# QData/LaMP

Measured on AMD Instinct MI355X. Metric: forward samples/sec, reuters d512 2+2L 4h, higher is better.
Workload: dtype f32

## Files before the change

### lamp_amd/csrc/chain.hip

```cpp
#include "lamp_asm.h"

namespace lamp {

namespace {
constexpr int ROWS = 16;
constexpr int BK = 32;

}

struct ChainGemm {
    const float* W[3];
    const float* Wp[3];
    const float* Wq[3];
    const float* bias[3];
    float* C[3];
    int nseg, N, K;
    int64_t ldw, ldc;
    int relu;
    int src;
    int dst;
    int add_dst;
};
struct ChainLN {
    const float* g;
// ... 453 lines not shown
    const int tid = threadIdx.x, lane = tid & 63;
    const int wave = __builtin_amdgcn_readfirstlane(tid >> 6);
    const int l15 = lane & 15, hi = lane >> 4;
    const int64_t row0 = int64_t(blockIdx.x) * ROWS;
    const int rows_m = int(p.M - row0 < ROWS ? p.M - row0 : ROWS);
    const unsigned lds0 = unsigned(reinterpret_cast<uintptr_t>((lds_ptr)smem));
    const int d = p.d, dff = p.has_ffn ? p.w1.N : 0;
    const int x_floats = ROWS * d, h_floats = ROWS * p.hw;
    const int c_floats = x_floats + h_floats;
    const int c_g1 = c_floats, c_be1 = c_g1 + d, c_g2 = c_be1 + d, c_be2 = c_g2 + d, c_b2 = c_be2 + d, c_b1 = c_b2 + d;
    const int c_res = c_b1 + dff, c_wout = c_res + (p.ln1.res ? ROWS * d : 0);
    auto buf_b = [&](int which) { return lds0 + (which ? unsigned(x_floats) * 4u : 0u); };
    auto buf_f = [&](int which) { return smem + (which ? x_floats : 0); };
    auto buf_w = [&](int which) { return which ? p.hw : d; };

    int pc = 0;
    auto first = [&]() { return (wave - pc) & (WAVES - 1); };
    auto load_rows = [&](const float* src, int64_t ld, int width, int which) {
        const __amdgpu_buffer_rsrc_t rs = rsrc_u(src + row0 * ld, (uint64_t(rows_m - 1) * uint64_t(ld) + uint64_t(width)) * 4u);
        const int ppr = width / 256, n = ROWS * ppr;
        float* dst = buf_f(which);
        const int rl = buf_w(which);
        for (int k = first(); k < n; k += WAVES) {
            const int r = k / ppr, part = k - r * ppr;
            const unsigned voff = unsigned(r) * unsigned(ld) * 4u + unsigned(part * 64 + (lane ^ r)) * 16u;
            lds_dma16(rs, dst + r * rl + part * 256, r < rows_m ? voff : OOB, 0);
        }
        pc += n;
    };
    auto load_vec = [&](const float* src, int n_floats, int at) {
        const __amdgpu_buffer_rsrc_t rs = rsrc_u(src, uint64_t(n_floats) * 4u);
        const int n = n_floats / 256;
        for (int k = first(); k < n; k += WAVES) lds_dma16(rs, smem + at + k * 256, unsigned(k * 64 + lane) * 16u, 0);
        pc += n;
    };
    auto load_mod_rows = [&](const float* table, int mod, int at) {
        const __amdgpu_buffer_rsrc_t rs = rsrc_u(table, uint64_t(mod) * uint64_t(d) * 4u);
        const int ppr = d / 256, n = ROWS * ppr;
        for (int k = first(); k < n; k += WAVES) {
            const int r = k / ppr, part = k - r * ppr;
            const unsigned src_row = unsigned(row0 + r) % unsigned(mod);
            lds_dma16(rs, smem + at + r * d + part * 256, r < rows_m ? (src_row * unsigned(d) + unsigned(part * 64 + lane) * 4u) * 4u : OOB, 0);
        }
        pc += n;
    };
    if (p.in_x) load_rows(p.in_x, d, d, 0);
    load_rows(p.in_h, p.ld_h, p.k_h, 1);
    load_vec(p.ln1.g, d, c_g1);
    load_vec(p.ln1.b, d, c_be1);
    if (p.ln1.res) load_mod_rows(p.ln1.res, p.ln1.r_mod, c_res);
    const ChainLN& lnl = p.has_ffn ? p.ln2 : p.ln1;
    if (p.has_ffn) {
        load_vec(p.ln2.g, d, c_g2);
        load_vec(p.ln2.b, d, c_be2);
        load_vec(p.w2.bias[0], d, c_b2);
        load_vec(p.w1.bias[0], dff, c_b1);
    }
    if (lnl.w_out) load_mod_rows(lnl.w_out, lnl.n_labels, c_wout);
    wait_vmcnt<0>();
    wg_barrier();

    unsigned a_off[2][2];
#pragma unroll
    for (int o = 0; o < 2; ++o)
#pragma unroll
        for (int c = 0; c < 2; ++c) a_off[o][c] = unsigned(((o * 8 + c * 4 + hi) ^ l15) << 4);

#ifdef LAMP_TUNING
    unsigned long long gt[3][4] = {};
    int gt_i = 0;
#endif
    auto gemm = [&](const ChainGemm& g, int bias_at) {
        CHAIN_STAMP(0);
        const int nk = g.K / BK, npass = g.N / PASS_COLS, total = npass * nk;
        const unsigned w_bytes = unsigned(g.N) * unsigned(g.K) * 4u;
        u32x4 rsW = raw_rsrc(g.Wp[0], w_bytes);
        unsigned f_voff[2][NB];
#pragma unroll
        for (int c = 0; c < 2; ++c)
#pragma unroll
            for (int j = 0; j < NB; ++j) f_voff[c][j] = unsigned((j * nk * 2 + c) * 256 + lane * 4) * 4u;
        const unsigned pass_jump = unsigned(PASS_COLS / 16 - 1) * unsigned(nk) * 2048u + 2048u;
        unsigned s_off = unsigned(wave * (WCOLS / 16)) * unsigned(nk) * 2048u;
        int pt = 0, p_kt = 0, p_wrap = 0;
        auto adv_a = [&]() { ++pt; ++p_kt; p_wrap = p_kt == nk ? 1 : 0; };
        auto adv_b = [&]() { s_off += p_wrap ? pass_jump : 2048u; p_kt = p_wrap ? 0 : p_kt; };
        auto adv_c = [&]() {
#if defined(CHAIN_ABL) && (CHAIN_ABL & 1)
            rsW[2] = 0u;
#else
            rsW[2] = pt < total ? w_bytes : 0u;
#endif
        };
        f32x4 F[DEPTH][2][NB], fa[2][2];
        unsigned a_cur[2][2];
        const unsigned src_b = buf_b(g.src) + unsigned(l15) * unsigned(buf_w(g.src)) * 4u;
#pragma unroll
        for (int o = 0; o < 2; ++o)
#pragma unroll
            for (int c = 0; c < 2; ++c) a_cur[o][c] = src_b + a_off[o][c];
        static_for<0, DEPTH - 1>([&](auto J) {
            constexpr int j = decltype(J)::value;
            sgpr_guard(rsW, s_off);
#pragma unroll
            for (int c = 0; c < 2; ++c)
#pragma unroll
                for (int jb = 0; jb < NB; ++jb) F[j][c][jb] = buffer_read16_untracked(rsW, f_voff[c][jb], s_off);
            adv_a(); adv_b(); adv_c();
        });
#pragma unroll
        for (int c = 0; c < 2; ++c) fa[0][c] = lds_read16(a_cur[0][c]);
        wait_vmcnt<(DEPTH - 2) * NL>();
        wait_lgkmcnt<0>();
        CHAIN_STAMP(1);
        for (int pass = 0; pass < npass; ++pass) {
            const int col0 = pass * PASS_COLS + wave * WCOLS;
            f32x4 acc[NB];
#pragma unroll
            for (int j = 0; j < NB; ++j) acc[j] = f32x4{0.f, 0.f, 0.f, 0.f};
            for (int kt0 = 0; kt0 < nk; kt0 += DEPTH) {
                const unsigned q_next = unsigned(kt0 + DEPTH == nk ? 0 : (kt0 + DEPTH) >> 1) * 256u;
                static_for<0, DEPTH>([&](auto J) {
                    constexpr int j = decltype(J)::value, set = j & 1, setn = (j + 1) & 1;
                    constexpr int jl = (j + DEPTH - 1) % DEPTH;
                    constexpr int a_imm = (j + 1 == DEPTH) ? 0 : ((j + 1) >> 1) * 256;
                    static_for<0, NMF>([&](auto I) {
                        constexpr int i = decltype(I)::value, c = i / (4 * NB), comp = (i % (4 * NB)) / NB, jb = i % NB;
#if !(defined(CHAIN_ABL) && (CHAIN_ABL & 2))
                        acc[jb] = __builtin_amdgcn_mfma_f32_16x16x4f32(F[j][c][jb][comp], fa[set][c][comp], acc[jb], 0, 0, 0);
#else
                        asm volatile("" ::"v"(F[j][c][jb]), "v"(fa[set][c]));
#endif
                        __builtin_amdgcn_sched_barrier(0);
                        if constexpr (i % 2 == 0 && i / 2 < NL) {
                            constexpr int li = i / 2;
#if !(defined(CHAIN_ABL) && (CHAIN_ABL & 16))
                            F[jl][li / NB][li % NB] = buffer_read16_untracked(rsW, f_voff[li / NB][li % NB], s_off);
#endif
                        } else if constexpr (i == 1 || i == 3) {
#if !(defined(CHAIN_ABL) && (CHAIN_ABL & 8))
                            fa[setn][i / 2] = lds_read16_off<a_imm>(a_cur[setn][i / 2]);
#endif
                        } else if constexpr (i == 2 * NL + 1) {
                            adv_a();
                        } else if constexpr (i == 2 * NL + 2) {
                            if constexpr (j == DEPTH - 2) {
                                a_cur[0][0] = src_b + a_off[0][0] + q_next;
                                a_cur[0][1] = src_b + a_off[0][1] + q_next;
                            } else if constexpr (j == DEPTH - 1) {
                                a_cur[1][0] = src_b + a_off[1][0] + q_next;
                                a_cur[1][1] = src_b + a_off[1][1] + q_next;
                            }
                        } else if constexpr (i == 2 * NL + 3) {
                            adv_b();
                        } else if constexpr (i == 2 * NL + 5) {
                            adv_c();
                        } else if constexpr (i == NMF - 1) {
                            asm volatile("s_waitcnt vmcnt(%0) lgkmcnt(0)" ::"n"((DEPTH - 2) * NL) : "memory");
                        }
                        __builtin_amdgcn_sched_barrier(0);
                    });
                });
            }
            if (pass + 1 == npass) wait_vmcnt<0>();
            static_for<0, DEPTH - 1>([&](auto J) {
#pragma unroll
                for (int c = 0; c < 2; ++c)
#pragma unroll
                    for (int jb = 0; jb < NB; ++jb) keep_alive(F[decltype(J)::value][c][jb]);
            });
#pragma unroll
            for (int c = 0; c < 2; ++c) keep_alive(fa[0][c]);
            CHAIN_STAMP(2);
            f32x4 bv[NB], rv[NB];
            unsigned at[NB];
#pragma unroll
            for (int j = 0; j < NB; ++j) {
                const int col = col0 + j * 16 + 4 * hi;
                at[j] = buf_b(g.dst) + unsigned(l15) * unsigned(buf_w(g.dst)) * 4u + unsigned(((col >> 2) ^ l15) << 4);
                bv[j] = lds_read16(bias_at >= 0 ? lds0 + unsigned(bias_at + col) * 4u : at[j]);
                rv[j] = lds_read16(at[j]);
            }
            wait_lgkmcnt<0>();
#pragma unroll
            for (int j = 0; j < NB; ++j) {
                settle(bv[j]);
                settle(rv[j]);
            }
#pragma unroll
            for (int j = 0; j < NB; ++j) {
                const f32x4 b = bias_at >= 0 ? bv[j] : f32x4{0.f, 0.f, 0.f, 0.f};
                float4 v = make_float4(acc[j][0] + b[0], acc[j][1] + b[1], acc[j][2] + b[2], acc[j][3] + b[3]);
                if (g.relu) v = make_float4(fmaxf(v.x, 0.f), fmaxf(v.y, 0.f), fmaxf(v.z, 0.f), fmaxf(v.w, 0.f));
                if (g.add_dst) v = make_float4(v.x + rv[j][0], v.y + rv[j][1], v.z + rv[j][2], v.w + rv[j][3]);
                lds_write16(at[j], f32x4{v.x, v.y, v.z, v.w});
            }
        }
        wait_vmcnt<0>();
        wg_barrier();
        CHAIN_STAMP(3);
#ifdef LAMP_TUNING
        ++gt_i;
#endif
    };

    auto layernorm = [&](const ChainLN& n, int g_at, int be_at) {
        const int nv = d / 4;
        int cq[NV];
#pragma unroll
        for (int i = 0; i < NV; ++i) cq[i] = lane + i * 64 < nv ? lane + i * 64 : nv - 1;
#pragma unroll
        for (int q = 0; q < RPW; ++q) {
            const int r = wave + q * WAVES;
            const bool live = r < rows_m;
            const int64_t row = row0 + (live ? r : 0);
            const unsigned row_b = lds0 + unsigned(r) * unsigned(d) * 4u;
            f32x4 raw[NV], gg[NV], bb[NV], rr[NV], ww[NV];
#pragma unroll
            for (int i = 0; i < NV; ++i) {
                const unsigned self = row_b + unsigned((cq[i] ^ r) << 4);
                raw[i] = lds_read16(self);
                gg[i] = lds_read16(lds0 + unsigned(g_at) * 4u + unsigned(cq[i]) * 16u);
                bb[i] = lds_read16(lds0 + unsigned(be_at) * 4u + unsigned(cq[i]) * 16u);
                rr[i] = lds_read16(n.res ? lds0 + unsigned(c_res + r * d) * 4u + unsigned(cq[i]) * 16u : self);
                ww[i] = lds_read16(n.w_out ? lds0 + unsigned(c_wout + r * d) * 4u + unsigned(cq[i]) * 16u : self);
            }
            wait_lgkmcnt<0>();
#pragma unroll
            for (int i = 0; i < NV; ++i) {
                settle(raw[i]); settle(gg[i]); settle(bb[i]); settle(rr[i]); settle(ww[i]);
            }
            float4 v[NV];
#pragma unroll
            for (int i = 0; i < NV; ++i) {
                const bool in = lane + i * 64 < nv;
                v[i] = in ? make_float4(raw[i].x, raw[i].y, raw[i].z, raw[i].w) : make_float4(0.f, 0.f, 0.f, 0.f);
                if (n.res && in) {
                    v[i].x += rr[i].x; v[i].y += rr[i].y; v[i].z += rr[i].z; v[i].w += rr[i].w;
                }
            }
            float mean, rstd;
            ln_row_stats<NV>(v, lane, nv, d, n.eps, mean, rstd);
            float4* yr = (n.y && live) ? reinterpret_cast<float4*>(n.y + row * d) : nullptr;
            float dot = 0.f;
#pragma unroll
            for (int i = 0; i < NV; ++i) {
                if (lane + i * 64 < nv) {
                    const float4 o = ln_row_apply(v[i], mean, rstd, make_float4(gg[i].x, gg[i].y, gg[i].z, gg[i].w),
                                                  make_float4(bb[i].x, bb[i].y, bb[i].z, bb[i].w));
                    lds_write16(row_b + unsigned((cq[i] ^ r) << 4), f32x4{o.x, o.y, o.z, o.w});
                    if (yr) yr[cq[i]] = o;
                    if (n.w_out) dot += dot4_nocontract(o, make_float4(ww[i].x, ww[i].y, ww[i].z, ww[i].w));
                }
            }
            if (n.w_out) {
                dot = wave64_sum(dot);
                if (lane == 0 && live) n.logits[row] = dot;
            }
        }
        wg_barrier();
    };

#ifdef LAMP_TUNING
    unsigned long long t[6] = {};
    const unsigned long long c_begin = __builtin_readcyclecounter();
    if (p.trace) t[0] = wall_clock64();
#endif
    gemm(p.fc, -1);
#ifdef LAMP_TUNING
    if (p.trace) t[1] = wall_clock64();
#endif
    layernorm(p.ln1, c_g1, c_be1);
#ifdef LAMP_TUNING
    if (p.trace) t[2] = wall_clock64();
#endif
    if (p.has_ffn) {
        gemm(p.w1, c_b1);
#ifdef LAMP_TUNING
        if (p.trace) t[3] = wall_clock64();
#endif
        gemm(p.w2, c_b2);
#ifdef LAMP_TUNING
        if (p.trace) t[4] = wall_clock64();
#endif
        layernorm(p.ln2, c_g2, c_be2);
    }
#ifdef LAMP_TUNING
    if (p.trace && tid == 0) {
        unsigned long long* o = p.trace + size_t(blockIdx.x) * 24;
        t[5] = wall_clock64();
        for (int i = 0; i < 6; ++i) o[i] = t[i];
        o[6] = __builtin_readcyclecounter() - c_begin;
        o[7] = __builtin_amdgcn_s_getreg((31 << 11) | 20);
        for (int gi = 0; gi < 3; ++gi)
            for (int k = 0; k < 4; ++k) o[8 + gi * 4 + k] = gt[gi][k] - c_begin;
    }
#endif
}


template <int NV, int G>
__global__ __launch_bounds__(512, 2) void chain_rows4_kernel(ChainParams p) {
    constexpr int WAVES = 8, R = 4 * G, DEPTH = 4, NMF = 16 * G, RPW = (R + WAVES - 1) / WAVES;
    extern __shared__ __attribute__((aligned(16))) float smem[];
    const int tid = threadIdx.x, lane = tid & 63;
    const int wave = __builtin_amdgcn_readfirstlane(tid >> 6);
    const int l3 = lane & 3;
    const int64_t row0 = int64_t(blockIdx.x) * R;
    const int rows_m = int(p.M - row0 < R ? p.M - row0 : R);
    const unsigned lds0 = unsigned(reinterpret_cast<uintptr_t>((lds_ptr)smem));
    const int d = p.d, dff = p.has_ffn ? p.w1.N : 0;
    const int x_floats = R * d, h_floats = R * p.hw;
    const int c_floats = x_floats + h_floats;
    const int c_g1 = c_floats, c_be1 = c_g1 + d, c_g2 = c_be1 + d, c_be2 = c_g2 + d, c_b2 = c_be2 + d, c_b1 = c_b2 + d;
    const int c_res = p.res_alias ? x_floats + p.k_h : c_b1 + dff, res_ld = p.res_alias ? p.hw : d;
    const int c_wout = p.wout_late ? x_floats : (p.res_alias ? c_b1 + dff : c_res + (p.ln1.res ? R * d : 0));
    auto buf_b = [&](int which) { return lds0 + (which ? unsigned(x_floats) * 4u : 0u); };
    auto buf_f = [&](int which) { return smem + (which ? x_floats : 0); };
    auto buf_w = [&](int which) { return which ? p.hw : d; };

    int pc = 0;
    auto first = [&]() { return (wave - pc) & (WAVES - 1); };
    auto load_rows = [&](const float* src, int64_t ld, int width, int which) {
        const __amdgpu_buffer_rsrc_t rs = rsrc_u(src + row0 * ld, (uint64_t(rows_m - 1) * uint64_t(ld) + uint64_t(width)) * 4u);
        const int ppr = width / 256, n = R * ppr;
        float* dst = buf_f(which);
        const int rl = buf_w(which);
        for (int k = first(); k < n; k += WAVES) {
            const int r = k / ppr, part = k - r * ppr;
            const unsigned voff = unsigned(r) * unsigned(ld) * 4u + unsigned(part * 64 + (lane ^ (r & 15))) * 16u;
            lds_dma16(rs, dst + r * rl + part * 256, r < rows_m ? voff : OOB, 0);
        }
        pc += n;
    };
    auto load_vec = [&](const float* src, int n_floats, int at) {
        const __amdgpu_buffer_rsrc_t rs = rsrc_u(src, uint64_t(n_floats) * 4u);
        const int n = n_floats / 256;
        for (int k = first(); k < n; k += WAVES) lds_dma16(rs, smem + at + k * 256, unsigned(k * 64 + lane) * 16u, 0);
        pc += n;
    };
    auto load_mod_rows = [&](const float* table, int mod, int at, int ld) {
        const __amdgpu_buffer_rsrc_t rs = rsrc_u(table, uint64_t(mod) * uint64_t(d) * 4u);
        const int ppr = d / 256, n = R * ppr;
        for (int k = first(); k < n; k += WAVES) {
            const int r = k / ppr, part = k - r * ppr;
            const unsigned src_row = unsigned(row0 + r) % unsigned(mod);
            lds_dma16(rs, smem + at + r * ld + part * 256, r < rows_m ? (src_row * unsigned(d) + unsigned(part * 64 + lane) * 4u) * 4u : OOB, 0);
        }
        pc += n;
    };
    if (p.in_x) load_rows(p.in_x, d, d, 0);
    load_rows(p.in_h, p.ld_h, p.k_h, 1);
    load_vec(p.ln1.g, d, c_g1);
    load_vec(p.ln1.b, d, c_be1);
    if (p.ln1.res) load_mod_rows(p.ln1.res, p.ln1.r_mod, c_res, res_ld);
    const ChainLN& lnl = p.has_ffn ? p.ln2 : p.ln1;
    if (p.has_ffn) {
        load_vec(p.ln2.g, d, c_g2);
        load_vec(p.ln2.b, d, c_be2);
        load_vec(p.w2.bias[0], d, c_b2);
        load_vec(p.w1.bias[0], dff, c_b1);
    }
    if (lnl.w_out && !p.wout_late) load_mod_rows(lnl.w_out, lnl.n_labels, c_wout, d);
    wait_vmcnt<0>();
    wg_barrier();

#ifdef LAMP_TUNING
    unsigned long long gt[3][4] = {};
    int gt_i = 0;
#endif
    auto gemm = [&](const ChainGemm& g, int bias_at) {
        CHAIN_STAMP(0);
        const int nc = g.K / 16, npass = g.N / 512, total = npass * nc;
        const unsigned w_bytes = unsigned(g.N) * unsigned(g.K) * 4u;
        u32x4 rsW = raw_rsrc(g.Wq[0], w_bytes);
        const unsigned f_voff = unsigned(lane) * 16u;
        const unsigned pass_jump = 7u * unsigned(nc) * 4096u + 4096u;
        unsigned s_off = unsigned(wave) * unsigned(nc) * 4096u;
        int pt = 0, p_kt = 0, p_wrap = 0;
        auto adv_a = [&]() { ++pt; ++p_kt; p_wrap = p_kt == nc ? 1 : 0; };
        auto adv_b = [&]() { s_off += p_wrap ? pass_jump : 4096u; p_kt = p_wrap ? 0 : p_kt; };
        auto adv_c = [&]() {
#if defined(CHAIN_ABL) && (CHAIN_ABL & 1)
            rsW[2] = 0u;
#else
            rsW[2] = pt < total ? w_bytes : 0u;
#endif
        };
        auto wload = [&](f32x4& dst, auto Q) { dst = buffer_read16_untracked_off<decltype(Q)::value * 1024>(rsW, f_voff, s_off); };
        f32x4 F[DEPTH][4];
        float fa[2][G];
        unsigned a_cur[G];
        const unsigned src_b = buf_b(g.src), row_bytes = unsigned(buf_w(g.src)) * 4u;
        const int bq = lane >> 4, be = (lane >> 2) & 3;
        auto a_lane = [&](int gg) { return src_b + unsigned(4 * gg + l3) * row_bytes + unsigned((bq ^ l3) << 4) + unsigned(be) * 4u; };
#pragma unroll
        for (int gg = 0; gg < G; ++gg) a_cur[gg] = a_lane(gg);
        auto aread = [&](auto SET, auto GG, auto J) {
            constexpr int set = decltype(SET)::value, gg = decltype(GG)::value, j = decltype(J)::value;
            fa[set][gg] = lds_read4_off<64 * (j ^ (gg & 3))>(a_cur[gg]);
        };
        static_for<0, DEPTH - 1>([&](auto J) {
            constexpr int j = decltype(J)::value;
            sgpr_guard(rsW, s_off);
            static_for<0, 4>([&](auto Q) { wload(F[j][decltype(Q)::value], Q); });
            adv_a(); adv_b(); adv_c();
        });
        static_for<0, G>([&](auto GG) { aread(std::integral_constant<int, 0>{}, GG, std::integral_constant<int, 0>{}); });
        wait_vmcnt<(DEPTH - 2) * 4>();
        wait_lgkmcnt<0>();
        CHAIN_STAMP(1);
        for (int pass = 0; pass < npass; ++pass) {
            const int col = pass * 512 + wave * 64 + lane;
            f32x4 acc[G];
#pragma unroll
            for (int gg = 0; gg < G; ++gg) acc[gg] = f32x4{0.f, 0.f, 0.f, 0.f};
            for (int kt0 = 0; kt0 < nc; kt0 += DEPTH) {
                const unsigned q_next = unsigned(kt0 + DEPTH == nc ? 0 : (kt0 + DEPTH) >> 2) * 256u;
                static_for<0, DEPTH>([&](auto J) {
                    constexpr int j = decltype(J)::value, set = j & 1, setn = (j + 1) & 1;
                    constexpr int jl = (j + DEPTH - 1) % DEPTH, jn = (j + 1) % DEPTH;
                    static_for<0, NMF>([&](auto I) {
                        constexpr int i = decltype(I)::value, jj = i / (4 * G), q = (i / G) % 4, gg = i % G;
#if !(defined(CHAIN_ABL) && (CHAIN_ABL & 2))
                        acc[gg] = __builtin_amdgcn_mfma_f32_4x4x1f32(fa[set][gg], F[j][q][jj], acc[gg], 4, 4 * q + jj, 0);
#endif
                        __builtin_amdgcn_sched_barrier(0);
                        if constexpr (i < 8 && i % 2 == 0) {
#if !(defined(CHAIN_ABL) && (CHAIN_ABL & 16))
                            wload(F[jl][i / 2], std::integral_constant<int, i / 2>{});
#endif
                        } else if constexpr (i < 2 * G && i % 2 == 1 && i != NMF - 1) {
#if !(defined(CHAIN_ABL) && (CHAIN_ABL & 8))
                            aread(std::integral_constant<int, setn>{}, std::integral_constant<int, i / 2>{}, std::integral_constant<int, jn>{});
#endif
                        } else if constexpr (i == 8) {
                            adv_a();
                        } else if constexpr (i == 10) {
                            adv_b();
                        } else if constexpr (i == 12) {
                            adv_c();
                        } else if constexpr (i >= 14 && i % 2 == 0 && (i - 14) / 2 < G && j == DEPTH - 2) {
                            a_cur[(i - 14) / 2] = a_lane((i - 14) / 2) + q_next;
                        } else if constexpr (i == NMF - 1) {
                            asm volatile("s_waitcnt vmcnt(%0) lgkmcnt(0)" ::"n"((DEPTH - 2) * 4) : "memory");
                        }
                        __builtin_amdgcn_sched_barrier(0);
                    });
                });
            }
            if (pass + 1 == npass) wait_vmcnt<0>();
            static_for<0, DEPTH - 1>([&](auto J) { static_for<0, 4>([&](auto Q) { keep_alive(F[decltype(J)::value][decltype(Q)::value]); }); });
            static_for<0, G>([&](auto GG) { keep_alive(fa[0][decltype(GG)::value]); });
            CHAIN_STAMP(2);
            const unsigned drow = unsigned(buf_w(g.dst)) * 4u;
            float rv[G][4];
            unsigned at[G][4];
#pragma unroll
            for (int gg = 0; gg < G; ++gg)
#pragma unroll
                for (int i = 0; i < 4; ++i) {
                    const int r = 4 * gg + i;
                    at[gg][i] = buf_b(g.dst) + unsigned(r) * drow + unsigned(((col >> 2) ^ (r & 15)) << 4) + unsigned(col & 3) * 4u;
                    rv[gg][i] = lds_read4(at[gg][i]);
                }
            float bias_v = lds_read4(bias_at >= 0 ? lds0 + unsigned(bias_at + col) * 4u : at[0][0]);
            wait_lgkmcnt<0>();
            settle(bias_v);
#pragma unroll
            for (int gg = 0; gg < G; ++gg)
#pragma unroll
                for (int i = 0; i < 4; ++i) settle(rv[gg][i]);
            const float bias = bias_at >= 0 ? bias_v : 0.f;
#pragma unroll
            for (int gg = 0; gg < G; ++gg)
#pragma unroll
                for (int i = 0; i < 4; ++i) {
                    float v = acc[gg][i] + bias;
                    if (g.relu) v = fmaxf(v, 0.f);
                    if (g.add_dst) v = v + rv[gg][i];
                    lds_write4(at[gg][i], v);
                }
        }
        wait_vmcnt<0>();
        wg_barrier();
        CHAIN_STAMP(3);
#ifdef LAMP_TUNING
        ++gt_i;
#endif
    };

    auto layernorm = [&](const ChainLN& n, int g_at, int be_at) {
        const int nv = d / 4;
        int cq[NV];
#pragma unroll
        for (int i = 0; i < NV; ++i) cq[i] = lane + i * 64 < nv ? lane + i * 64 : nv - 1;
#pragma unroll
        for (int q = 0; q < RPW; ++q) {
            const int r = wave + q * WAVES;
            if (r < R) {
                const bool live = r < rows_m;
                const int64_t row = row0 + (live ? r : 0);
                const unsigned row_b = lds0 + unsigned(r) * unsigned(d) * 4u;
                f32x4 raw[NV], gg[NV], bb[NV], rr[NV], ww[NV];
#pragma unroll
                for (int i = 0; i < NV; ++i) {
                    const unsigned self = row_b + unsigned((cq[i] ^ (r & 15)) << 4);
                    raw[i] = lds_read16(self);
                    gg[i] = lds_read16(lds0 + unsigned(g_at) * 4u + unsigned(cq[i]) * 16u);
                    bb[i] = lds_read16(lds0 + unsigned(be_at) * 4u + unsigned(cq[i]) * 16u);
                    rr[i] = lds_read16(n.res ? lds0 + unsigned(c_res + r * res_ld) * 4u + unsigned(cq[i]) * 16u : self);
                    ww[i] = lds_read16(n.w_out ? lds0 + unsigned(c_wout + r * d) * 4u + unsigned(cq[i]) * 16u : self);
                }
                wait_lgkmcnt<0>();
#pragma unroll
                for (int i = 0; i < NV; ++i) {
                    settle(raw[i]); settle(gg[i]); settle(bb[i]); settle(rr[i]); settle(ww[i]);
                }
                float4 v[NV];
#pragma unroll
                for (int i = 0; i < NV; ++i) {
                    const bool in = lane + i * 64 < nv;
                    v[i] = in ? make_float4(raw[i].x, raw[i].y, raw[i].z, raw[i].w) : make_float4(0.f, 0.f, 0.f, 0.f);
                    if (n.res && in) {
                        v[i].x += rr[i].x; v[i].y += rr[i].y; v[i].z += rr[i].z; v[i].w += rr[i].w;
                    }
                }
                float mean, rstd;
                ln_row_stats<NV>(v, lane, nv, d, n.eps, mean, rstd);
                float4* yr = (n.y && live) ? reinterpret_cast<float4*>(n.y + row * d) : nullptr;
                float dot = 0.f;
#pragma unroll
                for (int i = 0; i < NV; ++i) {
                    if (lane + i * 64 < nv) {
                        const float4 o = ln_row_apply(v[i], mean, rstd, make_float4(gg[i].x, gg[i].y, gg[i].z, gg[i].w),
                                                      make_float4(bb[i].x, bb[i].y, bb[i].z, bb[i].w));
                        lds_write16(row_b + unsigned((cq[i] ^ (r & 15)) << 4), f32x4{o.x, o.y, o.z, o.w});
                        if (yr) yr[cq[i]] = o;
                        if (n.w_out) dot += dot4_nocontract(o, make_float4(ww[i].x, ww[i].y, ww[i].z, ww[i].w));
                    }
                }
                if (n.w_out) {
                    dot = wave64_sum(dot);
                    if (lane == 0 && live) n.logits[row] = dot;
                }
            }
        }
        wg_barrier();
    };

#ifdef LAMP_TUNING
    unsigned long long t[6] = {};
    const unsigned long long c_begin = __builtin_readcyclecounter();
    if (p.trace) t[0] = wall_clock64();
#endif
    gemm(p.fc, -1);
#ifdef LAMP_TUNING
    if (p.trace) t[1] = wall_clock64();
#endif
    layernorm(p.ln1, c_g1, c_be1);
#ifdef LAMP_TUNING
    if (p.trace) t[2] = wall_clock64();
#endif
    if (p.has_ffn) {
        gemm(p.w1, c_b1);
#ifdef LAMP_TUNING
        if (p.trace) t[3] = wall_clock64();
#endif
        gemm(p.w2, c_b2);
#ifdef LAMP_TUNING
        if (p.trace) t[4] = wall_clock64();
#endif
        if (p.wout_late) {
            load_mod_rows(p.ln2.w_out, p.ln2.n_labels, c_wout, d);
            wait_vmcnt<0>();
            wg_barrier();
        }
        layernorm(p.ln2, c_g2, c_be2);
    }
#ifdef LAMP_TUNING
    if (p.trace && tid == 0) {
        unsigned long long* o = p.trace + size_t(blockIdx.x) * 24;
        t[5] = wall_clock64();
        for (int i = 0; i < 6; ++i) o[i] = t[i];
        o[6] = __builtin_readcyclecounter() - c_begin;
        o[7] = __builtin_amdgcn_s_getreg((31 << 11) | 20);
        for (int gi = 0; gi < 3; ++gi)
            for (int k = 0; k < 4; ++k) o[8 + gi * 4 + k] = gt[gi][k] - c_begin;
    }
#endif
}

#ifdef LAMP_TUNING
static unsigned long long* g_chain_trace = nullptr;
extern "C" __attribute__((visibility("default"))) void lamp_debug_set_chain_trace(unsigned long long* buf) { g_chain_trace = buf; }
static int g_chain_mode = -1;
extern "C" __attribute__((visibility("default"))) void lamp_debug_force_chain(int mode) { g_chain_mode = mode; }
static int g_chain_geom = -1;
extern "C" __attribute__((visibility("default"))) void lamp_debug_chain_geometry(int idx) { g_chain_geom = idx; }
#endif

#define LAMP_CHAIN_GEOMS(X) X(0, 16, 32, 2, 1) X(1, 8, 32, 4, 2) X(2, 8, 32, 2, 2) X(3, 8, 32, 4, 1) X(4, 8, 64, 2, 1) \
    X(5, 16, 32, 2, 0) X(6, 8, 64, 4, 0) X(7, 16, 32, 2, 3) X(8, 16, 32, 4, 3) X(9, 8, 64, 2, 3) X(10, 8, 64, 4, 3) \
    X(11, 16, 32, 2, 4) X(12, 16, 32, 4, 4) X(13, 8, 64, 2, 4) X(14, 8, 64, 4, 4)
#ifndef LAMP_CHAIN_PACKED_GEOM
#define LAMP_CHAIN_PACKED_GEOM 12
#endif
static bool chain_geom_packed(int idx) { return idx >= 7 && idx <= 20; }
static bool chain_geom_lds_operands(int idx) { return idx >= 11 && idx <= 14; }
#if LAMP_CHAIN_PACKED_GEOM == 11
#define LAMP_CHAIN_PACKED_CASE(X) X(11, 16, 32, 2, 4)
#elif LAMP_CHAIN_PACKED_GEOM == 12
#define LAMP_CHAIN_PACKED_CASE(X) X(12, 16, 32, 4, 4)
#elif LAMP_CHAIN_PACKED_GEOM == 13
#define LAMP_CHAIN_PACKED_CASE(X) X(13, 8, 64, 2, 4)
#else
#define LAMP_CHAIN_PACKED_CASE(X) X(14, 8, 64, 4, 4)
#endif
struct ChainGeomInfo {
    int waves, pass_cols, ring_floats;
};
static ChainGeomInfo chain_geom(int idx) {
    switch (idx) {
#define X(I, W, C, D, S) \
    case I: return ChainGeomInfo{W, ChainGeom<W, C, D, S>::PASS_COLS, ChainGeom<W, C, D, S>::RING_FLOATS};
        LAMP_CHAIN_GEOMS(X)
#undef X
        default: return ChainGeomInfo{0, 0, 0};
    }
}
static int chain_geom_index(bool have_pack = false) {
#ifdef LAMP_TUNING
    if (g_chain_geom >= 0) return (chain_geom_packed(g_chain_geom) && !have_pack) ? 0 : g_chain_geom;
#endif
    return have_pack ? LAMP_CHAIN_PACKED_GEOM : 0;
}

static int rows4_groups(int64_t M, int d, int k_h, int dff, bool has_ffn, const lamp_chain_pack* pk, bool res_mod, bool w_out,
                        int* res_alias = nullptr, int* wout_late = nullptr) {
    if (res_alias) *res_alias = 0;
    if (wout_late) *wout_late = 0;
    if (!pk || !pk->fc4 || (has_ffn && (!pk->w14 || !pk->w24))) return 0;
    int G = int((M + 4 * 256 - 1) / (4 * 256));
    bool forced = false;
#ifdef LAMP_TUNING
    if (g_chain_geom >= 15 && g_chain_geom <= 20) {
        G = g_chain_geom - 14;
        forced = true;
    } else if (g_chain_geom >= 0) {
        return 0;
    }
#endif
    if (G < 1 || G > 6 || (G == 4 && !forced) || M > int64_t(4 * G) * 65535 || d % 512 || k_h % 64 || (has_ffn && dff % 512)) return 0;
    const int hw = has_ffn ? (k_h > dff ? k_h : dff) : k_h;
    const size_t base = size_t(4 * G) * size_t(d + hw) + size_t(5) * d + size_t(has_ffn ? dff : 0), rows = size_t(4 * G) * d;
    const size_t limit = size_t(160) * 1024 / 4;
    if (base + (res_mod ? rows : 0) + (w_out ? rows : 0) <= limit) return G;
    const bool ra = res_mod && has_ffn && hw >= k_h + d, wl = w_out && has_ffn && size_t(4 * G) * hw >= rows;
    if (base + (res_mod && !ra ? rows : 0) + (w_out && !wl ? rows : 0) > limit) return 0;
    if (res_alias) *res_alias = ra;
    if (wout_late) *wout_late = wl;
    return G;
}

bool chain_applies(int64_t M, int d, int k_h, int dff, bool has_ffn, const lamp_chain_pack* pk, bool res_mod, bool w_out) {
#ifdef LAMP_NO_CHAIN
    (void)M; (void)d; (void)k_h; (void)dff; (void)has_ffn; (void)pk; (void)res_mod; (void)w_out;
    return false;
#else
    const ChainGeomInfo gi = chain_geom(chain_geom_index());
    const int hw = has_ffn ? (k_h > dff ? k_h : dff) : k_h;
    if (M <= 0 || gi.waves == 0 || d % gi.pass_cols || k_h % 256 || (has_ffn && (dff % gi.pass_cols || dff % 256)) || d % 256 || d > 512)
        return false;
    if (size_t(ROWS) * size_t(d + hw) * 4 + size_t(gi.ring_floats) * 4 > size_t(160) * 1024) return false;
#ifdef LAMP_TUNING
    if (g_chain_mode == 0) return false;
    if (g_chain_mode == 1) return true;
#endif
    const int64_t panels = (M + ROWS - 1) / ROWS;
    if (pk && pk->fc && (!has_ffn || (pk->w1 && pk->w2))) {
        if (rows4_groups(M, d, k_h, dff, has_ffn, pk, res_mod, w_out) > 0) return M >= 512;
        return panels > 128 && panels <= 256;
    }
    return panels > 128 && panels <= 256;
#endif
}

template <int NV, int WAVES, int WCOLS, int DEPTH, int NSLOT>
static int launch_chain_geom(const ChainParams& p, size_t lds, unsigned grid, hipStream_t s) {
    void (*kern)(ChainParams);
    if constexpr (NSLOT == 4) kern = chain_packed_kernel<NV, WAVES, WCOLS, DEPTH>;
    else kern = chain_kernel<NV, WAVES, WCOLS, DEPTH, NSLOT>;
    static AttrOnce once;
    if (int e = once.set(reinterpret_cast<const void*>(kern), 160 * 1024)) return e;
    hipLaunchKernelGGL(kern, dim3(grid), dim3(WAVES * 64), lds, s, p);
    return int(hipGetLastError());
}

int launch_chain(const float* A, int64_t lda, int k_h, const float* res, int64_t r_mod, int64_t M, int d, const float* w_fc,
                 const float* ln1_g, const float* ln1_b, const lamp_ffn_weights* ffn, int dff, float* y, const float* w_out,
                 int n_labels, float* logits, hipStream_t s, const lamp_chain_pack* pk) {
    if (!A || !w_fc || !ln1_g || !ln1_b || (!y && !w_out)) return LAMP_E_NULL;
    if (ffn && (!ffn->w1 || !ffn->b1 || !ffn->w2 || !ffn->b2 || !ffn->ln_g || !ffn->ln_b)) return LAMP_E_NULL;
    if (!chain_applies(M, d, k_h, dff, ffn != nullptr, pk, res != nullptr && r_mod > 0, w_out != nullptr)) return LAMP_E_UNSUPPORTED;
    if (!aligned16(A) || !aligned16(res) || !aligned16(w_fc) || !aligned16(ln1_g) || !aligned16(ln1_b) || !aligned16(y) ||
        !aligned16(w_out) || (lda & 3))
        return LAMP_E_ALIGN;
    if (ffn && (!aligned16(ffn->w1) || !aligned16(ffn->b1) || !aligned16(ffn->w2) || !aligned16(ffn->b2) || !aligned16(ffn->ln_g) ||
                !aligned16(ffn->ln_b)))
        return LAMP_E_ALIGN;
    const bool have_pack = pk && pk->fc && (!ffn || (pk->w1 && pk->w2));
    const bool have_pack4 = pk && pk->fc4 && (!ffn || (pk->w14 && pk->w24));
    if (have_pack && (!aligned16(pk->fc) || !aligned16(pk->w1) || !aligned16(pk->w2))) return LAMP_E_ALIGN;
    if (have_pack4 && (!aligned16(pk->fc4) || !aligned16(pk->w14) || !aligned16(pk->w24))) return LAMP_E_ALIGN;
    ChainParams p{};
    p.M = M; p.d = d; p.hw = ffn ? (k_h > dff ? k_h : dff) : k_h;
    p.in_x = (res && r_mod == 0) ? res : nullptr;
    p.in_h = A; p.ld_h = lda; p.k_h = k_h;
    auto step = [&](const float* W, const float* Wp, const float* Wq, const float* bias, int N, int K, int relu, int src, int dst, int add_dst) {
        ChainGemm g{};
        g.W[0] = W; g.Wp[0] = have_pack ? Wp : nullptr; g.Wq[0] = have_pack4 ? Wq : nullptr; g.bias[0] = bias;
        g.nseg = 1; g.N = N; g.K = K; g.ldw = K; g.ldc = 0; g.relu = relu; g.src = src; g.dst = dst; g.add_dst = add_dst;
        return g;
    };
    p.fc = step(w_fc, pk ? pk->fc : nullptr, pk ? pk->fc4 : nullptr, nullptr, d, k_h, 0, 1, 0, p.in_x ? 1 : 0);
    const bool last1 = ffn == nullptr;
    p.ln1 = ChainLN{ln1_g, ln1_b, 1e-5f, r_mod > 0 ? res : nullptr, int(r_mod), last1 ? y : nullptr, last1 ? w_out : nullptr, n_labels, logits};
    p.has_ffn = ffn ? 1 : 0;
    if (ffn) {
        p.w1 = step(ffn->w1, pk ? pk->w1 : nullptr, pk ? pk->w14 : nullptr, ffn->b1, dff, d, 1, 0, 1, 0);
        p.w2 = step(ffn->w2, pk ? pk->w2 : nullptr, pk ? pk->w24 : nullptr, ffn->b2, d, dff, 0, 1, 0, 1);
        p.ln2 = ChainLN{ffn->ln_g, ffn->ln_b, 1e-5f, nullptr, 0, y, w_out, n_labels, logits};
    }
    p.trace = nullptr;
#ifdef LAMP_TUNING
    p.trace = g_chain_trace;
#endif
    const double fl = 2.0 * double(M) * (double(d) * k_h + (ffn ? 2.0 * double(d) * dff : 0.0));
    const double by = 4.0 * (double(M) * (k_h + 2.0 * d) + double(d) * k_h + (ffn ? 2.0 * double(d) * dff : 0.0));
    const int nv = (d / 4 + 63) / 64;
    {
        const ChainLN& lnl = ffn ? p.ln2 : p.ln1;
        const int G = rows4_groups(M, d, k_h, dff, ffn != nullptr, have_pack4 ? pk : nullptr, p.ln1.res != nullptr, lnl.w_out != nullptr,
                                   &p.res_alias, &p.wout_late);
        const size_t lds4 = (size_t(4 * G) * size_t(p.d + p.hw) + size_t(5) * d + size_t(ffn ? dff : 0) +
                             (p.ln1.res && !p.res_alias ? size_t(4 * G) * d : 0) + (lnl.w_out && !p.wout_late ? size_t(4 * G) * d : 0)) * 4;
        if (G > 0) {
            ProfScope prof(LAMP_K_GEMM, fl, by, s);
            const unsigned grid4 = unsigned((M + 4 * G - 1) / (4 * G));
            void (*kern)(ChainParams) = nullptr;
            switch (nv * 10 + G) {
                case 11: kern = chain_rows4_kernel<1, 1>; break;
                case 12: kern = chain_rows4_kernel<1, 2>; break;
                case 13: kern = chain_rows4_kernel<1, 3>; break;
                case 14: kern = chain_rows4_kernel<1, 4>; break;
                case 15: kern = chain_rows4_kernel<1, 5>; break;
                case 16: kern = chain_rows4_kernel<1, 6>; break;
                case 21: kern = chain_rows4_kernel<2, 1>; break;
                case 22: kern = chain_rows4_kernel<2, 2>; break;
                case 23: kern = chain_rows4_kernel<2, 3>; break;
                case 24: kern = chain_rows4_kernel<2, 4>; break;
                case 25: kern = chain_rows4_kernel<2, 5>; break;
                case 26: kern = chain_rows4_kernel<2, 6>; break;
                default: return LAMP_E_UNSUPPORTED;
            }
            static AttrOnce once[12];
            if (int e = once[(nv - 1) * 6 + G - 1].set(reinterpret_cast<const void*>(kern), 160 * 1024)) return e;
            hipLaunchKernelGGL(kern, dim3(grid4), dim3(512), lds4, s, p);
            return int(hipGetLastError());
        }
#ifdef LAMP_TUNING
        if (g_chain_geom >= 15) return LAMP_E_UNSUPPORTED;
#endif
    }
    int gidx = chain_geom_index(have_pack);
    size_t lds = size_t(ROWS) * size_t(p.d + p.hw) * 4 + size_t(chain_geom(gidx).ring_floats) * 4;
    if (chain_geom_lds_operands(gidx)) {
        const ChainLN& lnl = ffn ? p.ln2 : p.ln1;
        const size_t with_ops = lds + (size_t(5) * d + size_t(ffn ? dff : 0) + (p.ln1.res ? size_t(ROWS) * d : 0) + (lnl.w_out ? size_t(ROWS) * d : 0)) * 4;
        if (with_ops <= size_t(160) * 1024) lds = with_ops;
        else gidx = 8;
    }
    ProfScope prof(LAMP_K_GEMM, fl, by, s);
    const unsigned grid = unsigned((M + ROWS - 1) / ROWS);
#define X(I, W, C, D, S) \
    case I: return nv <= 1 ? launch_chain_geom<1, W, C, D, S>(p, lds, grid, s) : launch_chain_geom<2, W, C, D, S>(p, lds, grid, s);
    switch (gidx) {
#ifdef LAMP_TUNING
        LAMP_CHAIN_GEOMS(X)
#else
        X(0, 16, 32, 2, 1)
        X(8, 16, 32, 4, 3)
        LAMP_CHAIN_PACKED_CASE(X)
#endif
        default: return LAMP_E_UNSUPPORTED;
    }
#undef X
}

template <int FORMAT>
__global__ __launch_bounds__(256) void pack_weight_kernel(const float* __restrict__ W, int N, int K, int64_t ldw, float* __restrict__ out) {
    const int64_t q = int64_t(blockIdx.x) * 256 + threadIdx.x;
    if (q >= int64_t(N) * K / 4) return;
    const int l = int(q & 63);
    float4 v;
    if constexpr (FORMAT == 0) {
        const int nk = K / BK, c = int((q >> 6) & 1);
        const int64_t st = q >> 7;
        const int kt = int(st % nk), cb = int(st / nk);
        v = *reinterpret_cast<const float4*>(W + int64_t(16 * cb + (l & 15)) * ldw + 32 * kt + 16 * c + 4 * (l >> 4));
    } else {
        const int nc = K / 16, qq = int((q >> 6) & 3);
        const int64_t st = q >> 8;
        const int ch = int(st % nc), cb = int(st / nc);
        v = *reinterpret_cast<const float4*>(W + int64_t(64 * cb + l) * ldw + 16 * ch + 4 * qq);
    }
    reinterpret_cast<float4*>(out)[q] = v;
}
int launch_pack_weight(const float* W, int N, int K, int64_t ldw, int format, float* out, hipStream_t s) {
    if (!W || !out) return LAMP_E_NULL;
    if (N <= 0 || K <= 0 || ldw < K) return LAMP_E_DIMS;
    if (format != 0 && format != 1) return LAMP_E_UNSUPPORTED;
    if (format == 0 ? (N % 16 || K % BK) : (N % 64 || K % 16)) return LAMP_E_UNSUPPORTED;
    if (!aligned16(W) || !aligned16(out) || (ldw & 3)) return LAMP_E_ALIGN;
    const int64_t n4 = int64_t(N) * K / 4;
    if (format == 0) hipLaunchKernelGGL(pack_weight_kernel<0>, dim3(unsigned((n4 + 255) / 256)), dim3(256), 0, s, W, N, K, ldw, out);
    else hipLaunchKernelGGL(pack_weight_kernel<1>, dim3(unsigned((n4 + 255) / 256)), dim3(256), 0, s, W, N, K, ldw, out);
    return int(hipGetLastError());
}

#ifdef LAMP_TUNING
extern "C" __attribute__((visibility("default"))) int lamp_debug_launch_chain(
    const float* A, long long lda, int k_h, const float* res, long long r_mod, long long M, int d, const float* w_fc,
    const float* ln1_g, const float* ln1_b, const float* w1, const float* b1, const float* w2, const float* b2,
    const float* ln2_g, const float* ln2_b, int dff, float* y, void* stream, const float* pk_fc, const float* pk_w1,
    const float* pk_w2, const float* pk_fc4, const float* pk_w14, const float* pk_w24) {
    lamp_ffn_weights f{};
    f.w1 = w1; f.b1 = b1; f.w2 = w2; f.b2 = b2; f.ln_g = ln2_g; f.ln_b = ln2_b;
    const lamp_chain_pack pk{pk_fc, pk_w1, pk_w2, pk_fc4, pk_w14, pk_w24};
    const int keep = g_chain_mode;
    g_chain_mode = 1;
    const int e = launch_chain(A, lda, k_h, res, r_mod, M, d, w_fc, ln1_g, ln1_b, w1 ? &f : nullptr, dff, y, nullptr, 0, nullptr,
                               hipStream_t(stream), (pk_fc || pk_fc4) ? &pk : nullptr);
    g_chain_mode = keep;
    return e;
}
#endif

}
```

Baseline: 45600.

## Prefetch next GEMM's weight fragments across chained GEMMs and layernorm

Moves the weight-fragment register pipeline out of the per-GEMM lambda so the first GEMM's prologue loads overlap the initial LDS row loads. Near the end of each GEMM, the buffer resource switches to the next GEMM's weights, so the prologue of fc→w1 and w1→w2 is already in flight during the epilogue and layernorm. This removes the per-GEMM pipeline fill and the trailing vmcnt drain. In exchange it adds register pressure, and correctness now depends on the in-flight loads and the resource switch being timed exactly.

Result: no change. 45840 (median of 6 runs) (+0.5%).

```diff
diff --git a/lamp_amd/csrc/chain.hip b/lamp_amd/csrc/chain.hip
--- a/lamp_amd/csrc/chain.hip
+++ b/lamp_amd/csrc/chain.hip
@@ -779,6 +779,7 @@
 template <int NV, int G>
 __global__ __launch_bounds__(512, 2) void chain_rows4_kernel(ChainParams p) {
     constexpr int WAVES = 8, R = 4 * G, DEPTH = 4, NMF = 16 * G, RPW = (R + WAVES - 1) / WAVES;
+    static_assert(2 * G < 13, "MFMA gap 13 of a step must be free of fragment reads (the stream switch, adv_next)");
     extern __shared__ __attribute__((aligned(16))) float smem[];
     const int tid = threadIdx.x, lane = tid & 63;
     const int wave = __builtin_amdgcn_readfirstlane(tid >> 6);
@@ -839,33 +840,53 @@
         load_vec(p.w1.bias[0], dff, c_b1);
     }
     if (lnl.w_out && !p.wout_late) load_mod_rows(lnl.w_out, lnl.n_labels, c_wout, d);
-    wait_vmcnt<0>();
+
+    f32x4 F[DEPTH][4];
+    const unsigned f_voff = unsigned(lane) * 16u;
+    {
+        const u32x4 rs = raw_rsrc(p.fc.Wq[0], unsigned(p.fc.N) * unsigned(p.fc.K) * 4u);
+        unsigned so = unsigned(wave) * unsigned(p.fc.K / 16) * 4096u;
+        static_for<0, DEPTH - 1>([&](auto J) {
+            sgpr_guard(rs, so);
+            static_for<0, 4>([&](auto Q) {
+                F[decltype(J)::value][decltype(Q)::value] = buffer_read16_untracked_off<decltype(Q)::value * 1024>(rs, f_voff, so);
+            });
+            so += 4096u;
+        });
+    }
+    wait_vmcnt<(DEPTH - 1) * 4>();
     wg_barrier();
 
 #ifdef LAMP_TUNING
     unsigned long long gt[3][4] = {};
     int gt_i = 0;
 #endif
-    auto gemm = [&](const ChainGemm& g, int bias_at) {
+    auto gemm = [&](const ChainGemm& g, int bias_at, const ChainGemm& nx, bool has_nx) {
         CHAIN_STAMP(0);
         const int nc = g.K / 16, npass = g.N / 512, total = npass * nc;
         const unsigned w_bytes = unsigned(g.N) * unsigned(g.K) * 4u;
         u32x4 rsW = raw_rsrc(g.Wq[0], w_bytes);
-        const unsigned f_voff = unsigned(lane) * 16u;
         const unsigned pass_jump = 7u * unsigned(nc) * 4096u + 4096u;
-        unsigned s_off = unsigned(wave) * unsigned(nc) * 4096u;
-        int pt = 0, p_kt = 0, p_wrap = 0;
+        unsigned s_off = unsigned(wave) * unsigned(nc) * 4096u + unsigned(DEPTH - 1) * 4096u;
+        int pt = DEPTH - 1, p_kt = DEPTH - 1, p_wrap = 0;
+        const u32x4 rsN = raw_rsrc(nx.Wq[0], has_nx ? unsigned(nx.N) * unsigned(nx.K) * 4u : 0u);
+        const unsigned n_off = __builtin_amdgcn_readfirstlane(unsigned(wave) * unsigned(nx.K / 16) * 4096u);
         auto adv_a = [&]() { ++pt; ++p_kt; p_wrap = p_kt == nc ? 1 : 0; };
         auto adv_b = [&]() { s_off += p_wrap ? pass_jump : 4096u; p_kt = p_wrap ? 0 : p_kt; };
         auto adv_c = [&]() {
 #if defined(CHAIN_ABL) && (CHAIN_ABL & 1)
             rsW[2] = 0u;
 #else
-            rsW[2] = pt < total ? w_bytes : 0u;
-#endif
+            rsW[2] = pt < total ? w_bytes : rsN[2];
+#endif
+        };
+        auto adv_next = [&]() {
+            const bool sw = pt == total;
+            rsW[0] = sw ? rsN[0] : rsW[0];
+            rsW[1] = sw ? rsN[1] : rsW[1];
+            s_off = sw ? n_off : s_off;
         };
         auto wload = [&](f32x4& dst, auto Q) { dst = buffer_read16_untracked_off<decltype(Q)::value * 1024>(rsW, f_voff, s_off); };
-        f32x4 F[DEPTH][4];
         float fa[2][G];
         unsigned a_cur[G];
         const unsigned src_b = buf_b(g.src), row_bytes = unsigned(buf_w(g.src)) * 4u;
@@ -877,12 +898,8 @@
             constexpr int set = decltype(SET)::value, gg = decltype(GG)::value, j = decltype(J)::value;
             fa[set][gg] = lds_read4_off<64 * (j ^ (gg & 3))>(a_cur[gg]);
         };
-        static_for<0, DEPTH - 1>([&](auto J) {
-            constexpr int j = decltype(J)::value;
-            sgpr_guard(rsW, s_off);
-            static_for<0, 4>([&](auto Q) { wload(F[j][decltype(Q)::value], Q); });
-            adv_a(); adv_b(); adv_c();
-        });
+        sgpr_guard(rsW, s_off);
+        sgpr_guard(rsN, n_off);
         static_for<0, G>([&](auto GG) { aread(std::integral_constant<int, 0>{}, GG, std::integral_constant<int, 0>{}); });
         wait_vmcnt<(DEPTH - 2) * 4>();
         wait_lgkmcnt<0>();
@@ -917,6 +934,8 @@
                             adv_b();
                         } else if constexpr (i == 12) {
                             adv_c();
+                        } else if constexpr (i == 13 && j == 0) {
+                            adv_next();
                         } else if constexpr (i >= 14 && i % 2 == 0 && (i - 14) / 2 < G && j == DEPTH - 2) {
                             a_cur[(i - 14) / 2] = a_lane((i - 14) / 2) + q_next;
                         } else if constexpr (i == NMF - 1) {
@@ -926,7 +945,7 @@
                     });
                 });
             }
-            if (pass + 1 == npass) wait_vmcnt<0>();
+            if (pass + 1 == npass && !has_nx) wait_vmcnt<0>();
             static_for<0, DEPTH - 1>([&](auto J) { static_for<0, 4>([&](auto Q) { keep_alive(F[decltype(J)::value][decltype(Q)::value]); }); });
             static_for<0, G>([&](auto GG) { keep_alive(fa[0][decltype(GG)::value]); });
             CHAIN_STAMP(2);
@@ -959,7 +978,6 @@
                     lds_write4(at[gg][i], v);
                 }
         }
-        wait_vmcnt<0>();
         wg_barrier();
         CHAIN_STAMP(3);
 #ifdef LAMP_TUNING
@@ -1031,7 +1049,7 @@
     const unsigned long long c_begin = __builtin_readcyclecounter();
     if (p.trace) t[0] = wall_clock64();
 #endif
-    gemm(p.fc, -1);
+    gemm(p.fc, -1, p.w1, p.has_ffn != 0);
 #ifdef LAMP_TUNING
     if (p.trace) t[1] = wall_clock64();
 #endif
@@ -1040,11 +1058,11 @@
     if (p.trace) t[2] = wall_clock64();
 #endif
     if (p.has_ffn) {
-        gemm(p.w1, c_b1);
+        gemm(p.w1, c_b1, p.w2, true);
 #ifdef LAMP_TUNING
         if (p.trace) t[3] = wall_clock64();
 #endif
-        gemm(p.w2, c_b2);
+        gemm(p.w2, c_b2, p.w2, false);
 #ifdef LAMP_TUNING
         if (p.trace) t[4] = wall_clock64();
 #endif
```
